# GabrieleCocco/CLFaceDetection

Measured on AMD Instinct MI355X. Metric: candidate windows/sec, 1080p, haarcascade_frontalface_alt, higher is better.
Workload: dtype u32 gathers + f32 stage sums; 1 GPU; BASELINE config 3: 64x1920x1080 8-bit frames per step in the whole job (noise/smooth/blocks mix; sharded by whole frames over 1 GPU), haarcascade_frontalface_alt, scaleFactor 1.1f, raw candidates, frames resident in HBM; frames_on_rank_0=64, windows_per_frame=6290352, parallelism=single GPU, device=AMD Radeon Graphics (gfx950:sramecc+:xnack-), 256 CUs, pipeline=vj_stream, two batches in flight

## Files before the change

### clfacedetection_amd/api.py

```python
from __future__ import annotations

import ctypes as C
import os
from dataclasses import dataclass

import numpy as np

from .build import LIB_PATH, build_lib

VJ_MAX_STAGES = 64
VJ_FLAG_COUNTERS = 1 << 0
VJ_FLAG_SIGNED_MEAN = 1 << 1
VJ_FLAG_SKIP_LIST = 1 << 2
VJ_FLAG_SKIP_ROW = 1 << 3
VJ_FLAG_GRID_F64 = 1 << 4
VJ_FLAG_TILTED_AS_UPRIGHT = 1 << 5
VJ_FLAG_CV_CANNY_PRUNING = 1 << 6
VJ_FLAG_CV_SCALE_IMAGE = 1 << 7
VJ_FLAG_CV_FIND_BIGGEST = 1 << 8
VJ_FLAG_CV_ROUGH_SEARCH = 1 << 9

CV_HAAR_DO_CANNY_PRUNING = 1
CV_HAAR_SCALE_IMAGE = 2
CV_HAAR_FIND_BIGGEST_OBJECT = 4
CV_HAAR_DO_ROUGH_SEARCH = 8

CLOD_PRECOMPUTE_FEATURES = 2 << 0
CLOD_BLOCK_IMPLEMENTATION = 2 << 1
CLOD_PER_STAGE_ITERATIONS = 2 << 2

DATA_DIR = os.path.join(os.path.dirname(os.path.abspath(__file__)), "data")


class VjError(RuntimeError):
    def __init__(self, code: int, what: str, detail: str):
        super().__init__(f"{what}: {detail}" if detail else what)
        self.code = code


class CascadeInfo(C.Structure):
    _fields_ = [(n, C.c_int32) for n in ("win_w", "win_h", "n_stages", "n_trees", "n_nodes", "n_alpha",
                                          "max_trees_per_stage", "max_nodes_per_tree", "n_tilted", "n_three_rect",
                                          "is_stump_based", "is_stage_tree")]


class Params(C.Structure):
    _fields_ = [("min_w", C.c_int32), ("min_h", C.c_int32), ("max_w", C.c_int32), ("max_h", C.c_int32),
                ("scale_factor", C.c_float), ("min_neighbors", C.c_uint32), ("flags", C.c_uint32),
                ("scale_mask", C.c_uint64 * 2)]


class ScaleInfo(C.Structure):
    _fields_ = [("scale_idx", C.c_int32), ("scale", C.c_float), ("step", C.c_float),
                ("win_w", C.c_int32), ("win_h", C.c_int32),
                ("equ_x", C.c_int32), ("equ_y", C.c_int32), ("equ_w", C.c_int32), ("equ_h", C.c_int32),
                ("area", C.c_uint32), ("nx", C.c_int32), ("ny", C.c_int32), ("accepted", C.c_int32)]


class _Image(C.Structure):
    _fields_ = [("data", C.c_void_p), ("width", C.c_int32), ("height", C.c_int32), ("stride", C.c_int32),
                ("on_device", C.c_int32), ("channels", C.c_int32)]


class CvParams(C.Structure):
    _fields_ = [("min_w", C.c_int32), ("min_h", C.c_int32), ("scale_factor", C.c_double), ("min_neighbors", C.c_uint32),
                ("flags", C.c_uint32)]


class CvPlanInfo(C.Structure):
    _fields_ = [("tile_windows", C.c_uint64), ("n_tile_scales", C.c_uint32), ("tree_prefix", C.c_uint32),
                ("tree_queue", C.c_int32), ("tq_shift", C.c_int32), ("tq_split_frames", C.c_int32), ("reserved", C.c_int32)]


class _Counters(C.Structure):
    _fields_ = [("windows", C.c_uint64), ("stump_evals", C.c_uint64), ("gather_bytes", C.c_uint64),
                ("stage_entered", C.c_uint64 * VJ_MAX_STAGES)]


VJ_MAX_PASSES = 8
VJ_MAX_LAUNCHES = 16
LAUNCH_KINDS = {0: "grid", 1: "queue", 2: "tile", 3: "block"}


class _Launch(C.Structure):
    _fields_ = [("kind", C.c_int32), ("lds_class", C.c_int32), ("stage_begin", C.c_int32), ("stage_end", C.c_int32),
                ("ms", C.c_float), ("lds_bytes", C.c_uint32), ("scale_mask", C.c_uint64 * 2),
                ("stage_entered", C.c_uint64 * VJ_MAX_STAGES)]


class _Timing(C.Structure):
    _fields_ = [("integral_ms", C.c_float), ("cascade_ms", C.c_float), ("total_ms", C.c_float),
                ("n_cascade_launches", C.c_int32), ("pass_ms", C.c_float * VJ_MAX_PASSES),
                ("pass_stage_begin", C.c_int32 * VJ_MAX_PASSES), ("pass_stage_end", C.c_int32 * VJ_MAX_PASSES),
                ("n_launches", C.c_int32), ("launch", _Launch * VJ_MAX_LAUNCHES), ("tile_split", C.c_float),
                ("balance_state", C.c_int32), ("balance_calls", C.c_int32)]


class _Result(C.Structure):
    _fields_ = [("rects", C.c_void_p), ("count", C.c_uint32), ("counters", _Counters), ("timing", _Timing)]


class CvRocParams(C.Structure):
    _fields_ = [("min_w", C.c_int32), ("min_h", C.c_int32), ("max_w", C.c_int32), ("max_h", C.c_int32),
                ("scale_factor", C.c_double), ("min_neighbors", C.c_uint32), ("flags", C.c_uint32)]


class _RocResult(C.Structure):
    _fields_ = [("r", _Result), ("reject_levels", C.c_void_p), ("level_weights", C.c_void_p)]


RECT_DTYPE = np.dtype([("x", "<i4"), ("y", "<i4"), ("w", "<i4"), ("h", "<i4"), ("weight", "<f4"),
                       ("frame", "<i4"), ("scale_idx", "<i4")])
STAGE_DTYPE = np.dtype([("first_tree", "<i4"), ("n_trees", "<i4"), ("threshold", "<f4"), ("parent", "<i4"),
                        ("next", "<i4"), ("child", "<i4")])
TREE_DTYPE = np.dtype([("first_node", "<i4"), ("n_nodes", "<i4"), ("first_alpha", "<i4")])
_RECT_DESC = np.dtype([("x", "<i4"), ("y", "<i4"), ("w", "<i4"), ("h", "<i4"), ("weight", "<f4")])
NODE_DTYPE = np.dtype([("n_rects", "<i4"), ("tilted", "<i4"), ("threshold", "<f4"), ("left", "<i4"),
                       ("right", "<i4"), ("rect", _RECT_DESC, 3)])

_SIGNATURES = {
    "vj_strerror": (C.c_char_p, [C.c_int]),
    "vj_last_error": (C.c_char_p, []),
    "vj_cascade_load_xml": (C.c_int, [C.c_char_p, C.POINTER(C.c_void_p)]),
    "vj_cascade_load": (C.c_int, [C.c_char_p, C.POINTER(C.c_void_p)]),
    "vj_cascade_save": (C.c_int, [C.c_void_p, C.c_char_p]),
    "vj_cascade_from_arrays": (C.c_int, [C.c_int, C.c_int, C.c_void_p, C.c_int, C.c_void_p, C.c_int, C.c_void_p, C.c_int,
                                         C.c_void_p, C.c_int, C.POINTER(C.c_void_p)]),
    "vj_cascade_free": (None, [C.c_void_p]),
    "vj_cascade_get_info": (C.c_int, [C.c_void_p, C.POINTER(CascadeInfo)]),
    "vj_cascade_stages": (C.c_void_p, [C.c_void_p]),
    "vj_cascade_trees": (C.c_void_p, [C.c_void_p]),
    "vj_cascade_nodes": (C.c_void_p, [C.c_void_p]),
    "vj_cascade_alpha": (C.c_void_p, [C.c_void_p]),
    "vj_cascade_notice": (C.c_char_p, [C.c_void_p]),
    "vj_params_default": (None, [C.POINTER(Params)]),
    "vj_plan_scales": (C.c_int, [C.c_void_p, C.c_int, C.c_int, C.POINTER(Params), C.POINTER(ScaleInfo), C.c_int,
                                 C.POINTER(C.c_int)]),
    "vj_plan_feature_table": (C.c_int, [C.c_void_p, C.c_int, C.POINTER(ScaleInfo), C.c_void_p, C.c_void_p]),
    "vj_env_create": (C.c_int, [C.c_int, C.POINTER(C.c_void_p)]),
    "vj_env_destroy": (None, [C.c_void_p]),
    "vj_env_reserve": (C.c_int, [C.c_void_p, C.c_int, C.c_int, C.c_int]),
    "vj_env_device_name": (C.c_int, [C.c_void_p, C.c_char_p, C.c_size_t]),
    "vj_env_configure": (C.c_int, [C.c_void_p, C.c_char_p, C.c_char_p]),
    "vj_env_query": (C.c_int, [C.c_void_p, C.c_char_p, C.c_char_p, C.c_size_t]),
    "vj_integral": (C.c_int, [C.c_void_p, C.c_void_p, C.c_int, C.c_int, C.c_int, C.c_void_p, C.c_void_p]),
    "vj_integral_image": (C.c_int, [C.c_void_p, C.c_void_p, C.c_void_p, C.c_void_p]),
    "vj_integral_tilted": (C.c_int, [C.c_void_p, C.c_void_p, C.c_void_p]),
    "vj_grayscale": (C.c_int, [C.c_void_p, C.c_void_p, C.c_void_p, C.c_int]),
    "vj_canny": (C.c_int, [C.c_void_p, C.c_void_p, C.c_void_p, C.c_int]),
    "vj_resize_linear": (C.c_int, [C.c_void_p, C.c_void_p, C.c_int, C.c_int, C.c_void_p, C.c_int]),
    "vj_host_alloc": (C.c_int, [C.c_void_p, C.c_size_t, C.POINTER(C.c_void_p)]),
    "vj_host_free": (None, [C.c_void_p, C.c_void_p]),
    "vj_detect_chain": (C.c_int, [C.c_void_p, C.c_void_p, C.c_void_p, C.POINTER(_Image), C.c_int, C.POINTER(Params),
                                  C.POINTER(Params), C.POINTER(_Result), C.POINTER(_Result)]),
    "vj_stream_create": (C.c_int, [C.c_void_p, C.c_void_p, C.c_int, C.c_int, C.c_int, C.c_int, C.POINTER(Params),
                                   C.POINTER(C.c_void_p)]),
    "vj_stream_submit": (C.c_int, [C.c_void_p, C.POINTER(_Image), C.c_int]),
    "vj_stream_collect": (C.c_int, [C.c_void_p, C.POINTER(_Result)]),
    "vj_stream_destroy": (None, [C.c_void_p]),
    "vj_detect_rois": (C.c_int, [C.c_void_p, C.c_void_p, C.POINTER(_Image), C.c_int, C.c_void_p, C.c_int, C.POINTER(Params),
                                 C.POINTER(_Result)]),
    "vj_detect_opencv": (C.c_int, [C.c_void_p, C.c_void_p, C.POINTER(_Image), C.c_int, C.POINTER(CvParams),
                                   C.POINTER(_Result)]),
    "vj_detect_opencv_rois": (C.c_int, [C.c_void_p, C.c_void_p, C.POINTER(_Image), C.c_int, C.c_void_p, C.c_int, C.POINTER(CvParams),
                                        C.POINTER(_Result)]),
    "vj_detect_opencv_chain": (C.c_int, [C.c_void_p, C.c_void_p, C.c_void_p, C.POINTER(_Image), C.c_int, C.POINTER(CvParams),
                                         C.POINTER(CvParams), C.POINTER(_Result), C.POINTER(_Result)]),
    "vj_cv_params_default": (None, [C.POINTER(CvParams)]),
    "vj_cv_roc_params_default": (None, [C.POINTER(CvRocParams)]),
    "vj_detect_opencv_roc": (C.c_int, [C.c_void_p, C.c_void_p, C.POINTER(_Image), C.c_int, C.POINTER(CvRocParams),
                                       C.POINTER(_RocResult)]),
    "vj_roc_result_free": (None, [C.POINTER(_RocResult)]),
    "vj_cv_plan_info_get": (C.c_int, [C.c_void_p, C.c_void_p, C.c_int, C.c_int, C.c_int, C.POINTER(CvParams), C.POINTER(CvPlanInfo)]),
    "vj_detect": (C.c_int, [C.c_void_p, C.c_void_p, C.POINTER(_Image), C.c_int, C.POINTER(Params),
                            C.POINTER(_Result)]),
    "vj_result_free": (None, [C.POINTER(_Result)]),
    "vj_group_rectangles": (C.c_int, [C.c_void_p, C.POINTER(C.c_uint32), C.c_int, C.c_double]),
    "vj_group_rectangles_levels": (C.c_int, [C.c_void_p, C.c_void_p, C.c_void_p, C.c_int, C.c_int, C.c_double]),
    "vj_count_windows": (C.c_int, [C.c_void_p, C.c_int, C.c_int, C.POINTER(Params), C.POINTER(C.c_uint64)]),
    "vj_shard_frames": (C.c_int, [C.c_int, C.c_int, C.c_int, C.POINTER(C.c_int), C.POINTER(C.c_int)]),
    "vj_shard_scales": (C.c_int, [C.c_void_p, C.c_int, C.c_int, C.POINTER(Params), C.c_int, C.c_int, C.POINTER(C.c_uint64)]),
}

_lib = None


def load_library(build: bool = True) -> C.CDLL:
    global _lib
    if _lib is not None:
        return _lib
    path = build_lib() if build else LIB_PATH
# ... 55 lines not shown
            return cls.load_xml(path)
        h = C.c_void_p()
        _check(load_library().vj_cascade_load(os.fsencode(path), C.byref(h)), f"vj_cascade_load({path})")
        return cls(h.value)

    @classmethod
    def from_arrays(cls, win_w: int, win_h: int, stages: np.ndarray, trees: np.ndarray, nodes: np.ndarray,
                    alpha: np.ndarray) -> "Cascade":
        st = np.ascontiguousarray(stages, STAGE_DTYPE)
        tr = np.ascontiguousarray(trees, TREE_DTYPE)
        nd = np.ascontiguousarray(nodes, NODE_DTYPE)
        al = np.ascontiguousarray(alpha, np.float32)
        h = C.c_void_p()
        _check(load_library().vj_cascade_from_arrays(int(win_w), int(win_h), st.ctypes.data, len(st), tr.ctypes.data, len(tr),
                                                     nd.ctypes.data, len(nd), al.ctypes.data, len(al), C.byref(h)),
               "vj_cascade_from_arrays")
        return cls(h.value)

    def save(self, path: str):
        _check(load_library().vj_cascade_save(self._h, os.fsencode(path)), f"vj_cascade_save({path})")

    def _view(self, fn, dtype, n):
        ptr = fn(self._h)
        buf = (C.c_char * (dtype.itemsize * n)).from_address(ptr)
        return np.frombuffer(buf, dtype, n).copy()

    @property
    def stages(self): return self._view(load_library().vj_cascade_stages, STAGE_DTYPE, self.info.n_stages)
    @property
    def trees(self): return self._view(load_library().vj_cascade_trees, TREE_DTYPE, self.info.n_trees)
    @property
    def nodes(self): return self._view(load_library().vj_cascade_nodes, NODE_DTYPE, self.info.n_nodes)
    @property
    def alpha(self): return self._view(load_library().vj_cascade_alpha, np.dtype("<f4"), self.info.n_alpha)
    @property
    def notice(self) -> str: return load_library().vj_cascade_notice(self._h).decode("latin-1")

    def plan_scales(self, width: int, height: int, params: Params | None = None) -> list[ScaleInfo]:
        p = params or default_params()
        n = C.c_int(0)
        lib = load_library()
        _check(lib.vj_plan_scales(self._h, width, height, C.byref(p), None, 0, C.byref(n)), "vj_plan_scales")
        arr = (ScaleInfo * max(n.value, 1))()
        _check(lib.vj_plan_scales(self._h, width, height, C.byref(p), arr, n.value, C.byref(n)), "vj_plan_scales")
        return list(arr)[:n.value]

    def feature_table(self, width: int, scale: ScaleInfo) -> tuple[np.ndarray, np.ndarray]:
        off = np.zeros((self.info.n_nodes, 3, 4), np.uint32)
        wts = np.zeros((self.info.n_nodes, 3), np.float32)
        _check(load_library().vj_plan_feature_table(self._h, width, C.byref(scale), off.ctypes.data,
                                                    wts.ctypes.data), "vj_plan_feature_table")
        return off, wts

    def shard_scales(self, width: int, height: int, rank: int, world: int, params: Params | None = None) -> list[int]:
        p = params or default_params()
        m = (C.c_uint64 * 2)()
        _check(load_library().vj_shard_scales(self._h, width, height, C.byref(p), world, rank, m), "vj_shard_scales")
        return [k for k in range(127) if (m[k >> 6] >> (k & 63)) & 1]

    def count_windows(self, width: int, height: int, params: Params | None = None) -> int:
        p = params or default_params()
        out = C.c_uint64(0)
        _check(load_library().vj_count_windows(self._h, width, height, C.byref(p), C.byref(out)), "vj_count_windows")
        return out.value

    def close(self):
        if self._h:
            load_library().vj_cascade_free(self._h)
            self._h = C.c_void_p()

    def __del__(self):
        try:
            self.close()
        except Exception:
            pass


@dataclass
class DetectResult:
    rects: np.ndarray
    windows: int
    stump_evals: int
    gather_bytes: int
    stage_entered: list
    integral_ms: float
    cascade_ms: float
    total_ms: float
    n_cascade_launches: int
    passes: list = None
    launches: list = None
    tile_split: float = 0.0
    balance_state: int = 0
    balance_calls: int = 0
    reject_levels: np.ndarray = None
    level_weights: np.ndarray = None

    @property
    def match_count(self) -> int:
        return len(self.rects)


class Environment:

    def __init__(self, device_index: int = 0):
        h = C.c_void_p()
        _check(load_library().vj_env_create(device_index, C.byref(h)), "vj_env_create")
# ... 379 lines not shown
```

### clfacedetection_amd/csrc/vj_env.cpp

```cpp
#include "vj_internal.hpp"
#include "vj_device.hpp"

#include <hip/hip_runtime_api.h>

#include <algorithm>
#include <climits>
#include <cmath>
#include <cstdint>
#include <cstdio>
#include <cstdlib>
#include <cstring>
#include <map>
#include <memory>
#include <string>
#include <tuple>

#include "vj_env_internal.hpp"

using namespace vj;

namespace vj {

static uint32_t f2u(float f) {
    uint32_t u;
    memcpy(&u, &f, 4);
    return u;
}

static constexpr uint32_t kSlackRows = 2;

uint32_t frame_elems_for(int W, int H) {
    uint64_t e = (uint64_t)(W + 1) * (uint64_t)(H + 1 + kSlackRows);
    e = (e + 63u) & ~(uint64_t)63u;
    return (uint32_t)e;
}

static std::vector<uint32_t> default_pass_bounds(const vj_cascade& c, const StageProgram& prog,
                                                 const std::vector<int>& override_, const std::vector<int>& cut_nodes) {
    const uint32_t n = (uint32_t)c.stages.size();
    std::vector<uint32_t> b{0};
    if (!override_.empty()) {
        for (int v : override_)
            if (v > (int)b.back() && v < (int)n) b.push_back((uint32_t)v);
    } else {
        uint32_t acc = 0;
        size_t ci = 0;
        for (uint32_t s = 0; s < n && ci < cut_nodes.size(); ++s) {
            acc += prog.n_nodes[s];
            if (acc >= (uint32_t)cut_nodes[ci] && s + 1 < n) {
                b.push_back(s + 1);
                while (ci < cut_nodes.size() && acc >= (uint32_t)cut_nodes[ci]) ++ci;
            }
        }
    }
    b.push_back(n);
    while (b.size() > (size_t)VJ_MAX_PASSES + 1) b.erase(b.end() - 2);
    return b;
}

struct TileThresholds {
    int min_windows, accept_windows, max_dwords_per_window;
};

static int build_plan(vj_env* e, const vj_cascade& c, int W, int H, const vj_params& p, Plan* pl, float tile_split,
                      const TileThresholds& thresholds, bool one_pass = false) {
    pl->tile_split = tile_split;
    if ((int)c.stages.size() > VJ_MAX_STAGES) {
        set_error("cascade has %zu stages; at most %d are supported", c.stages.size(), VJ_MAX_STAGES);
        return VJ_ERR_LIMIT;
    }
    if (!(p.flags & VJ_FLAG_TILTED_AS_UPRIGHT))
        for (const auto& nd : c.nodes)
            if (nd.tilted) {
                set_error("the cascade has tilted features: the clod profile would evaluate them as upright rectangles like the reference "
                          "(clod.cpp:448-492 never reads the flag) — pass VJ_FLAG_TILTED_AS_UPRIGHT for that, or use vj_detect_opencv");
                return VJ_ERR_UNSUPPORTED;
            }
    pl->prog = build_stage_program(c);
    const uint32_t skip_mode = p.flags & (VJ_FLAG_SKIP_LIST | VJ_FLAG_SKIP_ROW);
    pl->skip_mode = skip_mode;
    pl->pos_mode = (p.flags & VJ_FLAG_GRID_F64) ? (skip_mode == VJ_FLAG_SKIP_LIST ? 3u : 2u)
                                                : (skip_mode == VJ_FLAG_SKIP_ROW ? 1u : 0u);
    for (const auto& t : c.trees)
        if (t.n_nodes != 1) pl->trees = true;
    if (pl->trees) {
        pl->tree2 = true;
        for (const auto& t : c.trees) {
            if (t.n_nodes != 2) { pl->tree2 = false; break; }
            const vj_node_desc& n0 = c.nodes[t.first_node];
            const vj_node_desc& n1 = c.nodes[t.first_node + 1];
            const int kids = (n0.left > 0) + (n0.right > 0);
            if (kids != 1 || (n0.left > 0 ? n0.left : n0.right) != 1 || n1.left > 0 || n1.right > 0) {
                pl->tree2 = false;
                break;
            }
        }
    }
    for (size_t s = 0; s < c.stages.size(); ++s) {
        const bool linear = pl->prog.on_fail[s] == STAGE_REJECT &&
                            (pl->prog.on_pass[s] == (int)s + 1 ||
                             (pl->prog.on_pass[s] == STAGE_ACCEPT && s + 1 == c.stages.size()));
        if (!linear) pl->general = true;
    }
    std::vector<uint32_t> order;
    if (!stage_sweep_order(pl->prog, &order)) {
        set_error("stage links form a cycle");
        return VJ_ERR_UNSUPPORTED;
    }
    if (pl->general && e->general_prefix) {
        uint32_t P = 0;
        while (P + 1 < order.size() && order[P] == P && pl->prog.on_fail[P] == STAGE_REJECT &&
               pl->prog.on_pass[P] == (int)(P + 1) && order[P + 1] == P + 1)
            ++P;
        if (P >= 2) pl->general_prefix = P;
    }
    pl->scales_all = plan_scales(c, W, H, p);
    pl->frame_elems = frame_elems_for(W, H);
    const uint32_t stride = (uint32_t)W + 1u;
    const size_t n_nodes = c.nodes.size();

    uint32_t shape_header_bytes = TILE_LDS_HEADER;
    if (!pl->trees && !pl->general && e->tile_sp_begin < (int)c.stages.size()) {
        uint32_t mx = 0;
        for (size_t s = 0; s < c.stages.size(); ++s) mx = std::max(mx, pl->prog.n_nodes[s]);
        if (mx <= (uint32_t)TILE_SP_MAX_BLOCKS * TILE_SP_BLOCK) {
            pl->wave_tail = true;
            shape_header_bytes += ((2u * 14u * (TILE_SP_BLOCK + 1u) + 2u * mx + 3u) & ~3u) * 4u;
        }
    }
    const uint32_t tile_header_bytes = TILE_LDS_HEADER;
    std::vector<NodeRec> table;
    std::vector<uint32_t> pos_tab;
    std::vector<std::pair<uint32_t, uint32_t>> tile_reach;
    for (const vj_scale_info& si : pl->scales_all) {
        if (!si.accepted || si.nx <= 0 || si.ny <= 0) continue;
        if ((p.scale_mask[0] | p.scale_mask[1]) != 0) {
            const int k = si.scale_idx;
            if (k >= 127 || !((p.scale_mask[k >> 6] >> (k & 63)) & 1ull)) continue;
        }
        if (pl->scales.size() >= (size_t)MAX_SCALES) {
            set_error("more than %d scales", MAX_SCALES);
            return VJ_ERR_LIMIT;
        }
        ScaleDev sd;
        memset(&sd, 0, sizeof(sd));
        sd.step = si.step;
        sd.nx = (uint32_t)si.nx;
        sd.nwin = (uint32_t)si.nx * (uint32_t)si.ny;
        sd.e_lt = (uint32_t)si.equ_y * stride + (uint32_t)si.equ_x;
        sd.e_dw = (uint32_t)si.equ_w;
        sd.e_dh = (uint32_t)si.equ_h * stride;
        sd.area = (float)si.area;
        sd.table_first = (uint32_t)table.size();
        sd.scale_idx = (uint32_t)si.scale_idx;
        sd.scale_f = si.scale;
        sd.win_w = (uint32_t)si.win_w;
        sd.win_h = (uint32_t)si.win_h;
        sd.sq32 = e->sq32 && (uint64_t)sd.win_w * sd.win_h <= SQ32_MAX_AREA ? 1u : 0u;
        table.resize(table.size() + n_nodes);
        int rc = build_node_table(c, W, si, table.data() + sd.table_first);
        if (rc) return rc;
        const uint32_t x_max = (uint32_t)std::lrint((double)((float)(si.nx - 1) * si.step)) + (pl->pos_mode != 0u ? 1u : 0u);
        const uint32_t y_max = (uint32_t)std::lrint((double)((float)(si.ny - 1) * si.step)) + (pl->pos_mode != 0u ? 1u : 0u);
        uint32_t reach = sd.e_lt + sd.e_dh + sd.e_dw;
        for (size_t k = 0; k < n_nodes; ++k) {
            const NodeRec& r = table[sd.table_first + k];
            const uint32_t dw[3] = {r.dw01 & 0xffffu, r.dw01 >> 16, r.dw2_flags & 0xffffu};
            for (int q = 0; q < 3; ++q)
                if (q < 2 || r.w[2] != 0.0f) reach = std::max(reach, (r.lt[q] + r.dh[q] + dw[q]) / 4u);
        }
        reach += y_max * stride + x_max;
        pl->max_reach_elems = std::max(pl->max_reach_elems, reach);
        pl->windows_per_frame += sd.nwin;
        sd.ny = (uint32_t)si.ny;
        if (pl->pos_mode & 2u) {
            if (pos_tab.empty()) pos_tab.push_back(0u);
            sd.pos_base = (uint32_t)pos_tab.size();
            const double stepd = std::max(2.0, (double)si.scale);
            const int n_pos = std::max(si.nx, si.ny) + 1;
            for (int i = 0; i < n_pos; ++i)
                pos_tab.push_back((pl->pos_mode & 1u) ? (uint32_t)std::round((double)i * stepd) : (uint32_t)std::lrint((double)i * stepd));
        }

        uint32_t reach_x = (uint32_t)(si.equ_x + si.equ_w), reach_y = (uint32_t)(si.equ_y + si.equ_h);
        for (size_t k = 0; k < n_nodes; ++k) {
            const NodeRec& r = table[sd.table_first + k];
            const uint32_t dw[3] = {r.dw01 & 0xffffu, r.dw01 >> 16, r.dw2_flags & 0xffffu};
            for (int q = 0; q < 3; ++q)
                if (q < 2 || r.w[2] != 0.0f) {
                    const uint32_t lt = r.lt[q] / 4u;
                    reach_x = std::max(reach_x, lt % stride + dw[q] / 4u);
                    reach_y = std::max(reach_y, lt / stride + (r.dh[q] / 4u) / stride);
                }
        }
        if ((!pl->general || pl->general_prefix) && si.ny < 65536 && si.nx < 65536) {
            static const uint32_t kTw[] = {64, 48, 32, 24, 16, 12, 8}, kTh[] = {32, 24, 16, 12, 8, 6, 4};
            uint32_t best_cls = TILE_CLASSES, best_n = 0, b_tw = 0, b_th = 0, b_pitch = 0, b_rows = 0;
            for (uint32_t cls = 0; cls < TILE_CLASSES && best_n < (uint32_t)thresholds.min_windows; ++cls) {
                const int kb = e->tile_class_kb[cls];
                const uint32_t lds_cu = (160u - (uint32_t)e->tile_lds_reserve_kb) * 1024u;
                const uint64_t budget = kb < 0 ? ((lds_cu - 2048u) / (uint32_t)(-kb) - shape_header_bytes) & ~63ull
                                               : std::min<uint64_t>((uint64_t)kb * 1024u, 160u * 1024u - shape_header_bytes);
                for (uint32_t tw : kTw)
                    for (uint32_t th : kTh) {
                        const uint32_t nwt = tw * th;
                        if (nwt > TILE_WAVES * TILE_WAVE_CAP || nwt < 64 || nwt <= best_n) continue;
                        uint32_t pitch = (uint32_t)std::ceil((double)(tw - 1) * (double)si.step) + 3u + reach_x;
                        if (si.step != 2.0f) {
                            pitch = (pitch + 3u) & ~3u;
                            if (pitch % 32u == 0u) pitch += 4u;
                        } else {
                            pitch |= 1u;
                        }
                        const uint32_t rows = (uint32_t)std::ceil((double)(th - 1) * (double)si.step) + 3u + reach_y;
                        if ((uint64_t)pitch * rows * 4u > budget) continue;
                        if ((uint64_t)pitch * rows > (uint64_t)thresholds.max_dwords_per_window * nwt) continue;
                        best_cls = cls; best_n = nwt; b_tw = tw; b_th = th; b_pitch = pitch; b_rows = rows;
                    }
            }
            if (best_n != 0u && best_n >= (uint32_t)thresholds.accept_windows) {
                sd.tile_rw = 1;
                sd.tile_tw = b_tw;
                sd.tile_th = b_th;
                sd.tile_pitch = b_pitch;
                sd.tile_rows = b_rows;
                sd.tile_class = best_cls;
            }
        }
        if (sd.tile_rw) {
            sd.tile_table_first = (uint32_t)table.size();
            table.resize(table.size() + n_nodes);
            sd.tile_half = si.step == 2.0f ? (sd.tile_pitch + 1u) / 2u : 0u;
            if (getenv("VJ_DEBUG_PLAN"))
                fprintf(stderr, "vj plan: scale %d s=%.3f step=%.2f nx=%u ny=%u class %u tile %ux%u = %u windows, pitch %u rows %u (%u B)%s\n",
                        si.scale_idx, si.scale, si.step, sd.nx, sd.ny, sd.tile_class, sd.tile_tw, sd.tile_th, sd.tile_tw * sd.tile_th,
                        sd.tile_pitch, sd.tile_rows, sd.tile_pitch * sd.tile_rows * 4u, sd.tile_half ? " deinterleaved" : " x4");
            rc = build_node_table_stride(c, sd.tile_pitch, si, table.data() + sd.tile_table_first, sd.tile_half);
            if (rc) return rc;
            auto col = [&](uint32_t cx) { return sd.tile_half ? (cx & 1u) * sd.tile_half + (cx >> 1) : cx; };
            sd.te_lt = (uint32_t)si.equ_y * sd.tile_pitch + col((uint32_t)si.equ_x);
            sd.te_dw = (int32_t)col((uint32_t)(si.equ_x + si.equ_w)) - (int32_t)col((uint32_t)si.equ_x);
            sd.te_dh = (uint32_t)si.equ_h * sd.tile_pitch;
            sd.tiles_x = (sd.nx + sd.tile_tw - 1) / sd.tile_tw;
            sd.tile_row_end = sd.ny;
            sd.grp_table_first = sd.tile_table_first;
            sd.grp_te_lt = sd.te_lt;
            sd.grp_te_dh = sd.te_dh;
            sd.grp_te_dw = sd.te_dw;
        }
        pl->scales.push_back(sd);
        pl->scales_info.push_back(si);
        tile_reach.push_back({reach_x, reach_y});
    }
    if (pl->max_reach_elems >= pl->frame_elems) {
        set_error("feature reach %u exceeds the frame allocation %u", pl->max_reach_elems, pl->frame_elems);
        return VJ_ERR_LIMIT;
    }
    pl->tile_lead.resize(pl->scales.size());
    for (uint32_t slot = 0; slot < pl->scales.size(); ++slot) pl->tile_lead[slot] = slot;
    auto groupable = [&](uint32_t k) {
        const ScaleDev& sd = pl->scales[k];
        return sd.tile_rw != 0u && sd.tile_half != 0u && sd.step == 2.0f;
    };
    for (uint32_t g0 = 0; e->tile_group > 1 && g0 < pl->scales.size();) {
        if (!groupable(g0)) { ++g0; continue; }
        uint32_t g1 = g0 + 1;
        while (g1 < pl->scales.size() && g1 - g0 < (uint32_t)e->tile_group && groupable(g1) &&
               tile_reach[g1].first >= tile_reach[g1 - 1].first && tile_reach[g1].second >= tile_reach[g1 - 1].second)
            ++g1;
// ... 161 lines not shown
            std::vector<int> seg_first_pass;
            for (const Seg& sg : segs) {
                seg_first_pass.push_back((int)bounds.size() - 1);
                const uint32_t cut = sg.e - sg.b > 4 ? sg.b + 3 : sg.e;
                if (cut < sg.e) { bounds.push_back(cut); last.push_back(0); failq.push_back(0); }
                const uint32_t cut2 = e->seg_cut2 > 3 && sg.e - sg.b > (uint32_t)e->seg_cut2 + 4u && bounds.size() + 2 * (segs.size() - seg_first_pass.size()) + 1 < (size_t)VJ_MAX_PASSES
                                          ? sg.b + (uint32_t)e->seg_cut2 : sg.e;
                if (cut2 < sg.e) { bounds.push_back(cut2); last.push_back(0); failq.push_back(0); }
                bounds.push_back(sg.e); last.push_back(1); failq.push_back(0);
            }
            if (ok && !segs.empty() && bounds.size() - 1 <= (size_t)VJ_MAX_PASSES) {
                for (size_t k = 0; k < segs.size(); ++k) {
                    if (segs[k].fail_pos < 0) continue;
                    int target_pass = -1;
                    for (size_t t = 0; t < segs.size(); ++t)
                        if (segs[t].b == (uint32_t)segs[k].fail_pos) target_pass = seg_first_pass[t];
                    const int p_end = k + 1 < segs.size() ? seg_first_pass[k + 1] : (int)bounds.size() - 1;
                    for (int ps = seg_first_pass[k]; ps < p_end; ++ps) failq[(size_t)ps] = (uint8_t)target_pass;
                }
                pl->pass_bounds = bounds;
                pl->seg_last = last;
                pl->seg_fail = failq;
                bool chain_ok = segs.size() <= 4;
                for (size_t k = 0; k < segs.size() && chain_ok; ++k)
                    if (segs[k].fail_pos >= 0 && (k + 1 >= segs.size() || segs[k + 1].b != (uint32_t)segs[k].fail_pos)) chain_ok = false;
                if (chain_ok) {
                    pl->tile_n_seg = (uint32_t)segs.size();
                    for (size_t k = 0; k < segs.size(); ++k) {
                        pl->tile_seg_end[k] = segs[k].e;
                        if (segs[k].fail_pos >= 0) pl->tile_seg_chain |= 1u << k;
                    }
                }
            }
        }
    }
    pl->tile_end = std::min<uint32_t>((uint32_t)c.stages.size(), std::max<uint32_t>((uint32_t)e->tile_end, pl->pass_bounds[1]));
    if (pl->pass_bounds.size() == 2) pl->tile_end = pl->pass_bounds[1];
    for (uint32_t cls = 0; cls < TILE_CLASSES; ++cls) {
        pl->class_first[cls] = (uint32_t)pl->tile_units.size();
        for (uint32_t slot = 0; slot < pl->scales.size(); ++slot) {
            const uint32_t lead = pl->tile_lead[slot];
            const ScaleDev& L = pl->scales[lead];
            if (!pl->scales[slot].tile_rw || L.tile_class != cls || (slot > 0 && pl->tile_lead[slot - 1] == lead)) continue;
            uint32_t row_end = 0, nx = 0;
            for (uint32_t k = slot; k <= lead; ++k) {
                row_end = std::max(row_end, pl->scales[k].tile_row_end);
                nx = std::max(nx, pl->scales[k].nx);
            }
            for (uint32_t iy0 = 0; iy0 < row_end; iy0 += L.tile_th)
                for (uint32_t ix0 = 0; ix0 < nx; ix0 += L.tile_tw)
                    pl->tile_units.push_back(UnitDev{slot, ix0 | (iy0 << 16), lead > slot ? lead - slot + 1u : 0u, 0});
            pl->class_lds[cls] = std::max(pl->class_lds[cls], L.tile_pitch * L.tile_rows * 4u);
        }
        if (pl->class_lds[cls]) pl->class_lds[cls] += tile_header_bytes;
    }
    pl->class_first[TILE_CLASSES] = (uint32_t)pl->tile_units.size();
    const uint32_t lds_cu = (160u - (uint32_t)e->tile_lds_reserve_kb) * 1024u;
    for (uint32_t cls = 0; cls + 1 < TILE_CLASSES; ++cls) {
        const int ka = e->tile_class_kb[cls], kb = e->tile_class_kb[cls + 1];
        if (ka >= 0 || kb >= 0 || !pl->class_lds[cls] || !pl->class_lds[cls + 1]) continue;
        const uint32_t na = (uint32_t)(-ka), nb = (uint32_t)(-kb);
        if (na <= nb || na % nb != 0u) continue;
        const uint32_t ratio = na / nb;
        uint32_t big = std::max(pl->class_lds[cls + 1], ratio * pl->class_lds[cls]);
        big = (big + ratio * 1024u - 1u) / (ratio * 1024u) * (ratio * 1024u);
        if ((uint64_t)big * nb > lds_cu) continue;
        pl->class_lds[cls + 1] = big;
        pl->class_lds[cls] = big / ratio;
    }

    std::vector<UnitDev> skip_units, skip_segs;
    if (skip_mode) {
        if (pl->general) {
            set_error("the skip modes restate the reference's CPU loops, which run linear cascades only");
            return VJ_ERR_UNSUPPORTED;
        }
        uint32_t word = 0;
        for (uint32_t slot = 0; slot < pl->scales.size(); ++slot) {
            ScaleDev& sd = pl->scales[slot];
            sd.skip_base = word;
            if (skip_mode == VJ_FLAG_SKIP_ROW) {
                sd.skip_wpr = (sd.nx + 63u) / 64u;
                for (uint32_t iy = 0; iy < sd.ny; ++iy) {
                    skip_segs.push_back(UnitDev{slot, word, sd.skip_wpr, 0});
                    for (uint32_t ix0 = 0; ix0 < sd.nx; ix0 += 64u)
                        skip_units.push_back(UnitDev{slot, ix0 | (iy << 16), std::min<uint32_t>(64u, sd.nx - ix0), word++});
                }
            } else {
                sd.skip_wpr = 0;
                const uint32_t n_words = (sd.nwin + 63u) / 64u;
                skip_segs.push_back(UnitDev{slot, word, n_words, 0});
                for (uint32_t i0 = 0; i0 < sd.nwin; i0 += 64u)
                    skip_units.push_back(UnitDev{slot, i0, std::min<uint32_t>(64u, sd.nwin - i0), word++});
            }
        }
        pl->skip_frame_words = word;
        pl->n_skip_units = (uint32_t)skip_units.size();
        pl->n_skip_segs = (uint32_t)skip_segs.size();
    }

    int rc;
    if (!skip_units.empty()) {
        if ((rc = pl->d_skip_units.ensure(skip_units.size() * sizeof(UnitDev)))) return rc;
        if ((rc = pl->d_skip_segs.ensure(skip_segs.size() * sizeof(UnitDev)))) return rc;
        HIP_TRY(hipMemcpy(pl->d_skip_units.p, skip_units.data(), skip_units.size() * sizeof(UnitDev), hipMemcpyHostToDevice));
        HIP_TRY(hipMemcpy(pl->d_skip_segs.p, skip_segs.data(), skip_segs.size() * sizeof(UnitDev), hipMemcpyHostToDevice));
    }
    if ((rc = pl->d_table.ensure(std::max<size_t>(table.size(), 1) * sizeof(NodeRec)))) return rc;
    if ((rc = pl->d_scales.ensure(std::max<size_t>(pl->scales.size(), 1) * sizeof(ScaleDev)))) return rc;
    if ((rc = pl->d_stages.ensure(pl->stages.size() * sizeof(StageDev)))) return rc;
    if ((rc = pl->d_units.ensure(std::max<size_t>(pl->units.size(), 1) * sizeof(UnitDev)))) return rc;
    if ((rc = pl->d_tile_units.ensure(std::max<size_t>(pl->tile_units.size(), 1) * sizeof(UnitDev)))) return rc;
    if (!pos_tab.empty()) {
        if ((rc = pl->d_pos_tab.ensure(pos_tab.size() * sizeof(uint32_t)))) return rc;
        HIP_TRY(hipMemcpy(pl->d_pos_tab.p, pos_tab.data(), pos_tab.size() * sizeof(uint32_t), hipMemcpyHostToDevice));
    }
    if (!pl->unit_groups.empty()) {
        if ((rc = pl->d_unit_groups.ensure(pl->unit_groups.size() * sizeof(UnitDev)))) return rc;
        HIP_TRY(hipMemcpy(pl->d_unit_groups.p, pl->unit_groups.data(), pl->unit_groups.size() * sizeof(UnitDev), hipMemcpyHostToDevice));
    }
    if ((rc = pl->d_sp_blocks.ensure(std::max<size_t>(sp_blocks.size(), 1) * sizeof(SpBlock)))) return rc;
    if (!sp_blocks.empty())
        HIP_TRY(hipMemcpy(pl->d_sp_blocks.p, sp_blocks.data(), sp_blocks.size() * sizeof(SpBlock), hipMemcpyHostToDevice));
    if (!pl->tile_units.empty())
        HIP_TRY(hipMemcpy(pl->d_tile_units.p, pl->tile_units.data(), pl->tile_units.size() * sizeof(UnitDev),
                          hipMemcpyHostToDevice));
    if (!table.empty())
        HIP_TRY(hipMemcpy(pl->d_table.p, table.data(), table.size() * sizeof(NodeRec), hipMemcpyHostToDevice));
    HIP_TRY(hipMemcpy(pl->d_stages.p, pl->stages.data(), pl->stages.size() * sizeof(StageDev), hipMemcpyHostToDevice));
    if (!pl->units.empty())
        HIP_TRY(hipMemcpy(pl->d_units.p, pl->units.data(), pl->units.size() * sizeof(UnitDev), hipMemcpyHostToDevice));
    return VJ_OK;
}

static int layout_queues(Plan* pl, int frames, uint64_t* total_entries) {
    const uint64_t frames_per_part = frames >= (int)Q_PARTS ? ((uint64_t)frames + Q_PARTS - 1) / Q_PARTS : 1;
    uint64_t base = 0;
    for (ScaleDev& sd : pl->scales) {
        sd.q_base = (uint32_t)base;
        sd.q_cap = (uint32_t)((uint64_t)sd.nwin * frames_per_part);
        base += (uint64_t)sd.nwin * frames_per_part * std::min<uint64_t>(Q_PARTS, (uint64_t)frames);
    }
    *total_entries = base;
    if (base > 0xffffffffull) {
        set_error("survivor queue needs %llu entries", (unsigned long long)base);
        return VJ_ERR_LIMIT;
    }
    if (pl->frames_q != frames && !pl->scales.empty()) {
        HIP_TRY(hipMemcpy(pl->d_scales.p, pl->scales.data(), pl->scales.size() * sizeof(ScaleDev),
                          hipMemcpyHostToDevice));
        pl->frames_q = frames;
    }
    return VJ_OK;
// ... 137 lines not shown
    FILE* f = fopen(path, "w");
    if (!f) {
        set_error("cannot write %s", path);
        return VJ_ERR_IO;
    }
    for (const auto& kv : e->balance) {
        const vj_env::PlanKey& k = std::get<0>(kv.first);
        const vj_env::Balance& b = kv.second;
        fprintf(f, "vjbal1 %llx %d %d %d %d %d %d %x %llx %llx %x %d %.4f %d %d %u %u %d\n", (unsigned long long)std::get<0>(k), std::get<1>(k),
                std::get<2>(k), std::get<3>(k), std::get<4>(k), std::get<5>(k), std::get<6>(k), std::get<7>(k), (unsigned long long)std::get<8>(k),
                (unsigned long long)std::get<9>(k), std::get<10>(k), std::get<1>(kv.first), (double)b.best, b.phase == 4 ? 0 : b.thr, b.phase,
                b.calls_total, b.calls_on_candidate, b.calls);
    }
    fclose(f);
    return VJ_OK;
}

static int balance_import(vj_env* e, const char* path) {
    FILE* f = fopen(path, "r");
    if (!f) {
        set_error("cannot read %s", path);
        return VJ_ERR_IO;
    }
    char line[512];
    int n_bad = 0;
    while (fgets(line, sizeof(line), f)) {
        unsigned long long hash, m0, m1;
        int W, H, a, b2, c2, d, cls, thr, state = 3;
        unsigned sf, flags;
        double split;
        if (line[0] == '#' || line[0] == '\n') continue;
        if (sscanf(line, "vjbal1 %llx %d %d %d %d %d %d %x %llx %llx %x %d %lf %d %d", &hash, &W, &H, &a, &b2, &c2, &d, &sf, &m0, &m1, &flags, &cls,
                   &split, &thr, &state) < 14 || !(split >= 0.0 && split <= 3.0) || cls < 1) {
            ++n_bad;
            continue;
        }
        if (state == 0) continue;
        vj_env::Balance b;
        b.cur = b.best = (float)split;
        b.thr = thr ? 1 : 0;
        b.phase = 3;
        b.thr_tried = b.far_tried = true;
        b.last_used = ++e->balance_tick;
        e->balance[vj_env::BalanceKey(vj_env::PlanKey((uint64_t)hash, W, H, a, b2, c2, d, (uint32_t)sf, (uint64_t)m0, (uint64_t)m1, (uint32_t)flags, 0u), cls)] = b;
    }
    fclose(f);
    if (n_bad) {
        set_error("%s: %d lines are not balance records", path, n_bad);
        return VJ_ERR_PARSE;
    }
    return VJ_OK;
}

static int get_plan(vj_env* e, const vj_cascade* c, int W, int H, const vj_params& p, Plan** out, int n_frames = 1 << 20) {
    const vj_env::Balance* bal = balance_of(e, c, W, H, p, n_frames, false);
    const BalanceChoice choice = bal ? balance_choice(bal, n_frames) : BalanceChoice{e->split_for(n_frames, p), 0, false};
    const float split = choice.split;
    int small = small_frame_class(e, W, H, n_frames);
    if (small == 0 && choice.thr == 1 && !e->tile_thresholds_set) small = 3;
    const bool one_pass = n_frames <= e->one_pass_max_frames && (uint64_t)W * (uint64_t)H >= 800000ull;
    vj_env::PlanKey key(c->uid, W, H, p.min_w, p.min_h, p.max_w, p.max_h, f2u(p.scale_factor), p.scale_mask[0],
                        p.scale_mask[1], (p.flags & (VJ_FLAG_SKIP_LIST | VJ_FLAG_SKIP_ROW | VJ_FLAG_GRID_F64 | VJ_FLAG_TILTED_AS_UPRIGHT)) | ((uint32_t)small << 8) | ((uint32_t)one_pass << 12), f2u(split));
    auto it = e->plans.find(key);
    if (it != e->plans.end()) {
        it->second->last_used = ++e->plan_tick;
        *out = it->second.get();
        return VJ_OK;
    }
    if ((int)e->plans.size() >= std::max(2, e->plan_cache_max)) {
        HIP_TRY(hipStreamSynchronize(e->stream));
        if (e->stream2) HIP_TRY(hipStreamSynchronize(e->stream2));
        while ((int)e->plans.size() >= std::max(2, e->plan_cache_max)) {
            auto lru = e->plans.begin();
            for (auto i = e->plans.begin(); i != e->plans.end(); ++i)
                if (i->second->last_used < lru->second->last_used) lru = i;
            lru->second->release_device();
            e->plans.erase(lru);
        }
    }
    auto pl = std::make_unique<Plan>();
    TileThresholds th{e->tile_min_windows, e->tile_accept_windows, e->tile_max_dwords_per_window};
    if (small == 2) th = TileThresholds{64, 64, 8000};
    else if (small == 1) th = TileThresholds{256, 256, 2000};
    else if (small == 3) th = TileThresholds{std::min(384, th.min_windows), std::min(384, th.accept_windows), th.max_dwords_per_window};
    int rc = build_plan(e, *c, W, H, p, pl.get(), split, th, one_pass);
    if (rc) {
        pl->release_device();
        return rc;
    }
    pl->last_used = ++e->plan_tick;
    *out = pl.get();
    e->plans[key] = std::move(pl);
    return VJ_OK;
}

int Lane::create() {
    for (auto& x : ev) HIP_TRY(hipEventCreate(&x));
    for (auto& x : pass_ev) HIP_TRY(hipEventCreate(&x));
    for (auto& x : launch_ev) HIP_TRY(hipEventCreate(&x));
    HIP_TRY(hipEventCreateWithFlags(&upload_done, hipEventDisableTiming));
    HIP_TRY(hipEventCreateWithFlags(&integral_done, hipEventDisableTiming));
    HIP_TRY(hipEventCreateWithFlags(&done, hipEventDisableTiming));
    h_pinned_bytes = (size_t)1 << 20;
    HIP_TRY(hipHostMalloc(&h_pinned, h_pinned_bytes, hipHostMallocDefault));
    return VJ_OK;
}

void Lane::destroy() {
    for (DevBuf* b : {&d_gray, &d_counts, &d_det}) b->release();
    if (h_pinned) (void)hipHostFree(h_pinned);
    if (h_stage) (void)hipHostFree(h_stage);
    h_pinned = h_stage = nullptr;
    for (auto& x : ev) if (x) (void)hipEventDestroy(x);
    for (auto& x : pass_ev) if (x) (void)hipEventDestroy(x);
    for (auto& x : launch_ev) if (x) (void)hipEventDestroy(x);
    for (hipEvent_t* x : {&upload_done, &integral_done, &done}) if (*x) (void)hipEventDestroy(*x);
}

int ensure_image_buffers(vj_env* e, int W, int H, int frames, bool need_gray, int channels, Lane* lane) {
    if (!lane) lane = &e->lane0;
    const size_t fe = frame_elems_for(W, H);
    const uint32_t n_bands = ((uint32_t)H + BAND_ROWS - 1) / BAND_ROWS;
    const uint32_t band_pitch = ((uint32_t)W + 3u) & ~3u;
    int rc;
    const size_t sum_bytes = fe * 4 * (size_t)frames, sq_bytes = fe * 8 * (size_t)frames;
    const bool grow = sum_bytes > e->d_sum.cap || sq_bytes > e->d_sqsum.cap;
    if ((rc = e->d_sum.ensure(sum_bytes))) return rc;
    if ((rc = e->d_sqsum.ensure(sq_bytes))) return rc;
    (void)grow;
    if (need_gray) {
        const size_t gstride = ((size_t)W * (size_t)channels + 3) & ~(size_t)3;
        if ((rc = lane->d_gray.ensure(gstride * (size_t)H * (size_t)frames))) return rc;
    }
    const size_t band_elems = (size_t)frames * n_bands * band_pitch;
    if ((rc = e->d_band_sum.ensure(band_elems * 4))) return rc;
    if ((rc = e->d_band_sq.ensure(band_elems * 4))) return rc;
    if ((rc = e->d_band_sqp.ensure(band_elems * 8))) return rc;
    return VJ_OK;
// ... 1870 lines not shown
    vj_env* e = s->e;
    HIP_TRY(hipSetDevice(e->device));
    const int lane = s->n_pending == 0 ? 0 : 1 - s->fifo[0];
    Lane* L = &s->lanes[lane];
    HIP_TRY(hipEventSynchronize(L->integral_done));
    if ((rc = enqueue_prepare(e, L, s->plan.get(), frames, n_frames, W, H, true, s->copy))) return rc;
    if ((rc = enqueue_cascade(e, L, s->plan.get(), W, H, s->p))) return rc;
    s->fifo[s->n_pending] = lane;
    s->n_frames_of[lane] = n_frames;
    s->n_pending++;
    return VJ_OK;
}

int vj_stream_collect(vj_stream* s, vj_result* out) {
    if (!s || !out) return VJ_ERR_ARG;
    memset(out, 0, sizeof(*out));
    if (s->n_pending == 0) {
        set_error("no batch is pending");
        return VJ_ERR_ARG;
    }
    vj_env* e = s->e;
    HIP_TRY(hipSetDevice(e->device));
    const int lane = s->fifo[0];
    s->fifo[0] = s->fifo[1];
    s->n_pending--;
    Lane* L = &s->lanes[lane];
    std::vector<RawDet> dets;
    int rc = finish_batch(e, L, s->plan.get(), 0, s->W, s->H, s->p, &dets, &out->counters, &out->timing);
    if (rc) return rc;
    return build_result(s->plan.get(), dets, s->n_frames_of[lane], s->p, out);
}

void vj_stream_destroy(vj_stream* s) {
    if (!s) return;
    (void)hipSetDevice(s->e->device);
    if (s->e->stream) (void)hipStreamSynchronize(s->e->stream);
    if (s->e->stream2) (void)hipStreamSynchronize(s->e->stream2);
    if (s->copy) {
        (void)hipStreamSynchronize(s->copy);
        (void)hipStreamDestroy(s->copy);
    }
    for (Lane& L : s->lanes) L.destroy();
    if (s->plan) s->plan->release_device();
    delete s;
}

void vj_result_free(vj_result* r) {
    if (!r) return;
    free(r->rects);
    r->rects = nullptr;
    r->count = 0;
}

}
```

### include/vj.h

```cpp
#ifndef VJ_H_
#define VJ_H_

#include <stdint.h>
#include <stddef.h>

#ifdef __cplusplus
extern "C" {
#endif
#if defined(VJ_BUILDING) && defined(__GNUC__)
#pragma GCC visibility push(default)
#endif

enum {
    VJ_OK = 0,
    VJ_ERR_ARG = 1,
    VJ_ERR_IO = 2,
    VJ_ERR_PARSE = 3,
    VJ_ERR_UNSUPPORTED = 4,
    VJ_ERR_NO_DEVICE = 5,
    VJ_ERR_HIP = 6,
    VJ_ERR_NOMEM = 7,
    VJ_ERR_LIMIT = 8
};
const char* vj_strerror(int code);
// ... 32 lines not shown
int  vj_cascade_load_xml(const char* path, vj_cascade** out);
int  vj_cascade_load(const char* path, vj_cascade** out);
int  vj_cascade_save(const vj_cascade* c, const char* path);
int  vj_cascade_from_arrays(int win_w, int win_h, const vj_stage_desc* stages, int n_stages,
                            const vj_tree_desc* trees, int n_trees, const vj_node_desc* nodes, int n_nodes,
                            const float* alpha, int n_alpha, vj_cascade** out);
void vj_cascade_free(vj_cascade* c);
int  vj_cascade_get_info(const vj_cascade* c, vj_cascade_info* out);
const vj_stage_desc* vj_cascade_stages(const vj_cascade* c);
const vj_tree_desc*  vj_cascade_trees(const vj_cascade* c);
const vj_node_desc*  vj_cascade_nodes(const vj_cascade* c);
const float*         vj_cascade_alpha(const vj_cascade* c);
const char*          vj_cascade_notice(const vj_cascade* c);

enum {
    VJ_FLAG_COUNTERS     = 1u << 0,
    VJ_FLAG_SIGNED_MEAN  = 1u << 1,
    VJ_FLAG_SKIP_LIST    = 1u << 2,
    VJ_FLAG_SKIP_ROW     = 1u << 3,
    VJ_FLAG_GRID_F64     = 1u << 4,
    VJ_FLAG_TILTED_AS_UPRIGHT = 1u << 5,
    VJ_FLAG_CV_CANNY_PRUNING = 1u << 6,
    VJ_FLAG_CV_SCALE_IMAGE = 1u << 7,
    VJ_FLAG_CV_FIND_BIGGEST = 1u << 8,
    VJ_FLAG_CV_ROUGH_SEARCH = 1u << 9,
};

typedef struct vj_params {
    int32_t  min_w, min_h;
    int32_t  max_w, max_h;
    float    scale_factor;
    uint32_t min_neighbors;
    uint32_t flags;
    uint64_t scale_mask[2];
} vj_params;
#define VJ_SCALE_MASK_NONE (1ull << 63)
void vj_params_default(vj_params* p);

typedef struct vj_scale_info {
    int32_t  scale_idx;
    float    scale;
    float    step;
    int32_t  win_w, win_h;
    int32_t  equ_x, equ_y, equ_w, equ_h;
    uint32_t area;
    int32_t  nx, ny;
    int32_t  accepted;
} vj_scale_info;
int vj_plan_scales(const vj_cascade* c, int width, int height, const vj_params* p,
                   vj_scale_info* out, int cap, int* n);

int vj_plan_feature_table(const vj_cascade* c, int width, const vj_scale_info* s,
                          uint32_t* offsets, float* weights);

typedef struct vj_env vj_env;
int  vj_env_create(int device_index, vj_env** out);
void vj_env_destroy(vj_env* e);
int  vj_env_reserve(vj_env* e, int max_w, int max_h, int max_batch);
int  vj_env_device_name(const vj_env* e, char* buf, size_t cap);
int  vj_env_configure(vj_env* e, const char* key, const char* value);
int  vj_env_query(const vj_env* e, const char* key, char* buf, size_t cap);

int vj_integral(vj_env* e, const uint8_t* gray, int w, int h, int stride,
                uint32_t* sum, uint64_t* sqsum);

int  vj_host_alloc(vj_env* e, size_t bytes, void** out);
void vj_host_free(vj_env* e, void* p);

struct vj_image;
int  vj_integral_image(vj_env* e, const struct vj_image* image, uint32_t* sum, uint64_t* sqsum);
int  vj_grayscale(vj_env* e, const struct vj_image* image, uint8_t* gray, int gray_stride);
int  vj_integral_tilted(vj_env* e, const struct vj_image* image, uint32_t* tilted);
int  vj_canny(vj_env* e, const struct vj_image* image, uint8_t* edges, int edges_stride);
int  vj_resize_linear(vj_env* e, const struct vj_image* image, int dst_w, int dst_h, uint8_t* dst, int dst_stride);
typedef struct vj_image {
    const uint8_t* data;
    int32_t width, height;
    int32_t stride;
    int32_t on_device;
    int32_t channels;
} vj_image;

typedef struct vj_rect {
    int32_t x, y, w, h;
    float   weight;
    int32_t frame;
    int32_t scale_idx;
} vj_rect;

#define VJ_MAX_STAGES 64
typedef struct vj_counters {
    uint64_t windows;
    uint64_t stump_evals;
    uint64_t gather_bytes;
    uint64_t stage_entered[VJ_MAX_STAGES];
} vj_counters;

#define VJ_MAX_PASSES 8
#define VJ_MAX_LAUNCHES 16
enum { VJ_LAUNCH_GRID = 0,
       VJ_LAUNCH_QUEUE = 1,
       VJ_LAUNCH_TILE = 2,
       VJ_LAUNCH_BLOCK = 3 };
typedef struct vj_launch {
    int32_t  kind;
    int32_t  lds_class;
// ... 106 lines not shown
```

Before: 10.47 billion windows/s.

## Widen LDS tile shape search and drop wave-tail header from tile budget

```diff
diff --git a/clfacedetection_amd/api.py b/clfacedetection_amd/api.py
--- a/clfacedetection_amd/api.py
+++ b/clfacedetection_amd/api.py
@@ -55,6 +55,22 @@
                 ("win_w", C.c_int32), ("win_h", C.c_int32),
                 ("equ_x", C.c_int32), ("equ_y", C.c_int32), ("equ_w", C.c_int32), ("equ_h", C.c_int32),
                 ("area", C.c_uint32), ("nx", C.c_int32), ("ny", C.c_int32), ("accepted", C.c_int32)]
+
+
+class TileInfo(C.Structure):
+    _fields_ = [("scale_idx", C.c_int32), ("scale", C.c_float), ("step", C.c_float), ("nx", C.c_int32), ("ny", C.c_int32),
+                ("lds_class", C.c_int32), ("tile_w", C.c_int32), ("tile_h", C.c_int32), ("pitch", C.c_int32), ("rows", C.c_int32),
+                ("reach_x", C.c_int32), ("reach_y", C.c_int32), ("lead_scale_idx", C.c_int32), ("tile_row_end", C.c_int32)]
+
+
+class TilePlanInfo(C.Structure):
+    _fields_ = [("header_bytes", C.c_uint32), ("gather_reserve_bytes", C.c_uint32), ("max_tile_windows", C.c_uint32),
+                ("n_classes", C.c_uint32), ("class_lds", C.c_uint32 * 4), ("class_per_cu", C.c_int32 * 4),
+                ("class_tiles", C.c_uint32 * 4)]
+
+
+VJ_PLAN_TILES_FORMER_SHAPES = 1
+VJ_PLAN_TILES_NO_GROUPS = 2
 
 
 class _Image(C.Structure):
@@ -137,6 +153,8 @@
     "vj_plan_scales": (C.c_int, [C.c_void_p, C.c_int, C.c_int, C.POINTER(Params), C.POINTER(ScaleInfo), C.c_int,
                                  C.POINTER(C.c_int)]),
     "vj_plan_feature_table": (C.c_int, [C.c_void_p, C.c_int, C.POINTER(ScaleInfo), C.c_void_p, C.c_void_p]),
+    "vj_plan_tiles": (C.c_int, [C.c_void_p, C.c_int, C.c_int, C.POINTER(Params), C.c_int, C.c_uint32, C.POINTER(TilePlanInfo),
+                                C.POINTER(TileInfo), C.c_int, C.POINTER(C.c_int)]),
     "vj_env_create": (C.c_int, [C.c_int, C.POINTER(C.c_void_p)]),
     "vj_env_destroy": (None, [C.c_void_p]),
     "vj_env_reserve": (C.c_int, [C.c_void_p, C.c_int, C.c_int, C.c_int]),
@@ -298,6 +316,18 @@
                                                     wts.ctypes.data), "vj_plan_feature_table")
         return off, wts
 
+    def plan_tiles(self, width: int, height: int, n_frames: int = 64, params: Params | None = None,
+                   flags: int = 0) -> tuple[TilePlanInfo, list[TileInfo]]:
+        p = params or default_params()
+        n = C.c_int(0)
+        info = TilePlanInfo()
+        lib = load_library()
+        _check(lib.vj_plan_tiles(self._h, width, height, C.byref(p), n_frames, flags, None, None, 0, C.byref(n)), "vj_plan_tiles")
+        arr = (TileInfo * max(n.value, 1))()
+        _check(lib.vj_plan_tiles(self._h, width, height, C.byref(p), n_frames, flags, C.byref(info), arr, n.value, C.byref(n)),
+               "vj_plan_tiles")
+        return info, list(arr)[:n.value]
+
     def shard_scales(self, width: int, height: int, rank: int, world: int, params: Params | None = None) -> list[int]:
         p = params or default_params()
         m = (C.c_uint64 * 2)()
diff --git a/clfacedetection_amd/csrc/vj_env.cpp b/clfacedetection_amd/csrc/vj_env.cpp
--- a/clfacedetection_amd/csrc/vj_env.cpp
+++ b/clfacedetection_amd/csrc/vj_env.cpp
@@ -62,8 +62,14 @@
     int min_windows, accept_windows, max_dwords_per_window;
 };
 
-static int build_plan(vj_env* e, const vj_cascade& c, int W, int H, const vj_params& p, Plan* pl, float tile_split,
-                      const TileThresholds& thresholds, bool one_pass = false) {
+struct PlanBuildOptions {
+    bool upload = true;
+    bool former_shapes = false;
+    std::vector<std::pair<uint32_t, uint32_t>>* tile_reach = nullptr;
+};
+
+static int build_plan(const vj_env* e, const vj_cascade& c, int W, int H, const vj_params& p, Plan* pl, float tile_split,
+                      const TileThresholds& thresholds, bool one_pass = false, const PlanBuildOptions& opt = PlanBuildOptions()) {
     pl->tile_split = tile_split;
     if ((int)c.stages.size() > VJ_MAX_STAGES) {
         set_error("cascade has %zu stages; at most %d are supported", c.stages.size(), VJ_MAX_STAGES);
@@ -119,16 +125,16 @@
     const uint32_t stride = (uint32_t)W + 1u;
     const size_t n_nodes = c.nodes.size();
 
-    uint32_t shape_header_bytes = TILE_LDS_HEADER;
+    const uint32_t tile_header_bytes = TILE_LDS_HEADER;
+    uint32_t shape_header_bytes = tile_header_bytes;
     if (!pl->trees && !pl->general && e->tile_sp_begin < (int)c.stages.size()) {
         uint32_t mx = 0;
         for (size_t s = 0; s < c.stages.size(); ++s) mx = std::max(mx, pl->prog.n_nodes[s]);
         if (mx <= (uint32_t)TILE_SP_MAX_BLOCKS * TILE_SP_BLOCK) {
             pl->wave_tail = true;
-            shape_header_bytes += ((2u * 14u * (TILE_SP_BLOCK + 1u) + 2u * mx + 3u) & ~3u) * 4u;
-        }
-    }
-    const uint32_t tile_header_bytes = TILE_LDS_HEADER;
+            if (opt.former_shapes) shape_header_bytes += ((2u * 14u * (TILE_SP_BLOCK + 1u) + 2u * mx + 3u) & ~3u) * 4u;
+        }
+    }
     std::vector<NodeRec> table;
     std::vector<uint32_t> pos_tab;
     std::vector<std::pair<uint32_t, uint32_t>> tile_reach;
@@ -194,7 +200,8 @@
                 }
         }
         if ((!pl->general || pl->general_prefix) && si.ny < 65536 && si.nx < 65536) {
-            static const uint32_t kTw[] = {64, 48, 32, 24, 16, 12, 8}, kTh[] = {32, 24, 16, 12, 8, 6, 4};
+            static const uint32_t kTw[] = {64, 56, 48, 40, 32, 24, 16, 12, 8}, kTh[] = {32, 28, 24, 20, 16, 12, 8, 6, 4};
+            auto former = [&](uint32_t v) { return opt.former_shapes && (v == 56u || v == 40u || v == 28u || v == 20u); };
             uint32_t best_cls = TILE_CLASSES, best_n = 0, b_tw = 0, b_th = 0, b_pitch = 0, b_rows = 0;
             for (uint32_t cls = 0; cls < TILE_CLASSES && best_n < (uint32_t)thresholds.min_windows; ++cls) {
                 const int kb = e->tile_class_kb[cls];
@@ -204,7 +211,8 @@
                 for (uint32_t tw : kTw)
                     for (uint32_t th : kTh) {
                         const uint32_t nwt = tw * th;
-                        if (nwt > TILE_WAVES * TILE_WAVE_CAP || nwt < 64 || nwt <= best_n) continue;
+                        if (nwt > TILE_WAVES * TILE_WAVE_CAP || nwt < 64 || nwt < best_n || (nwt == best_n && best_cls != cls)) continue;
+                        if (former(tw) || former(th)) continue;
                         uint32_t pitch = (uint32_t)std::ceil((double)(tw - 1) * (double)si.step) + 3u + reach_x;
                         if (si.step != 2.0f) {
                             pitch = (pitch + 3u) & ~3u;
@@ -215,6 +223,7 @@
                         const uint32_t rows = (uint32_t)std::ceil((double)(th - 1) * (double)si.step) + 3u + reach_y;
                         if ((uint64_t)pitch * rows * 4u > budget) continue;
                         if ((uint64_t)pitch * rows > (uint64_t)thresholds.max_dwords_per_window * nwt) continue;
+                        if (nwt == best_n && (opt.former_shapes || pitch * rows >= b_pitch * b_rows)) continue;
                         best_cls = cls; best_n = nwt; b_tw = tw; b_th = th; b_pitch = pitch; b_rows = rows;
                     }
             }
@@ -482,6 +491,9 @@
                     pl->tile_units.push_back(UnitDev{slot, ix0 | (iy0 << 16), lead > slot ? lead - slot + 1u : 0u, 0});
             pl->class_lds[cls] = std::max(pl->class_lds[cls], L.tile_pitch * L.tile_rows * 4u);
         }
+        for (const ScaleDev& sd : pl->scales)
+            if (sd.tile_rw && sd.tile_class == cls && pl->class_lds[cls])
+                pl->class_lds[cls] = std::max(pl->class_lds[cls], sd.tile_pitch * sd.tile_rows * 4u);
         if (pl->class_lds[cls]) pl->class_lds[cls] += tile_header_bytes;
     }
     pl->class_first[TILE_CLASSES] = (uint32_t)pl->tile_units.size();
@@ -529,6 +541,8 @@
         pl->n_skip_segs = (uint32_t)skip_segs.size();
     }
 
+    if (opt.tile_reach) *opt.tile_reach = tile_reach;
+    if (!opt.upload) return VJ_OK;
     int rc;
     if (!skip_units.empty()) {
         if ((rc = pl->d_skip_units.ensure(skip_units.size() * sizeof(UnitDev)))) return rc;
@@ -772,6 +786,14 @@
     return VJ_OK;
 }
 
+static TileThresholds thresholds_for(const vj_env* e, int small) {
+    TileThresholds th{e->tile_min_windows, e->tile_accept_windows, e->tile_max_dwords_per_window};
+    if (small == 2) th = TileThresholds{64, 64, 8000};
+    else if (small == 1) th = TileThresholds{256, 256, 2000};
+    else if (small == 3) th = TileThresholds{std::min(384, th.min_windows), std::min(384, th.accept_windows), th.max_dwords_per_window};
+    return th;
+}
+
 static int get_plan(vj_env* e, const vj_cascade* c, int W, int H, const vj_params& p, Plan** out, int n_frames = 1 << 20) {
     const vj_env::Balance* bal = balance_of(e, c, W, H, p, n_frames, false);
     const BalanceChoice choice = bal ? balance_choice(bal, n_frames) : BalanceChoice{e->split_for(n_frames, p), 0, false};
@@ -799,11 +821,7 @@
         }
     }
     auto pl = std::make_unique<Plan>();
-    TileThresholds th{e->tile_min_windows, e->tile_accept_windows, e->tile_max_dwords_per_window};
-    if (small == 2) th = TileThresholds{64, 64, 8000};
-    else if (small == 1) th = TileThresholds{256, 256, 2000};
-    else if (small == 3) th = TileThresholds{std::min(384, th.min_windows), std::min(384, th.accept_windows), th.max_dwords_per_window};
-    int rc = build_plan(e, *c, W, H, p, pl.get(), split, th, one_pass);
+    int rc = build_plan(e, *c, W, H, p, pl.get(), split, thresholds_for(e, small), one_pass);
     if (rc) {
         pl->release_device();
         return rc;
@@ -2780,4 +2798,61 @@
     r->count = 0;
 }
 
-}
+int vj_plan_tiles(const vj_cascade* c, int width, int height, const vj_params* p, int n_frames, uint32_t flags,
+                  vj_tile_plan_info* info, vj_tile_info* out, int cap, int* n) {
+    if (!c || !p || !n || width <= 0 || height <= 0 || n_frames <= 0 || (cap > 0 && !out) ||
+        (flags & ~(uint32_t)(VJ_PLAN_TILES_FORMER_SHAPES | VJ_PLAN_TILES_NO_GROUPS)))
+        return VJ_ERR_ARG;
+    int rc = check_params(*p);
+    if (rc) return rc;
+    auto e = std::make_unique<vj_env>();
+    if (flags & VJ_PLAN_TILES_NO_GROUPS) e->tile_group = 1;
+    Plan pl;
+    PlanBuildOptions opt;
+    std::vector<std::pair<uint32_t, uint32_t>> reach;
+    opt.upload = false;
+    opt.former_shapes = (flags & VJ_PLAN_TILES_FORMER_SHAPES) != 0u;
+    opt.tile_reach = &reach;
+    const bool one_pass = n_frames <= e->one_pass_max_frames && (uint64_t)width * (uint64_t)height >= 800000ull;
+    rc = build_plan(e.get(), *c, width, height, *p, &pl, e->split_for(n_frames, *p),
+                    thresholds_for(e.get(), small_frame_class(e.get(), width, height, n_frames)), one_pass, opt);
+    if (rc) return rc;
+    if (info) {
+        memset(info, 0, sizeof(*info));
+        info->header_bytes = TILE_LDS_HEADER;
+        info->gather_reserve_bytes = (uint32_t)e->tile_lds_reserve_kb * 1024u;
+        info->max_tile_windows = TILE_WAVES * TILE_WAVE_CAP;
+        info->n_classes = TILE_CLASSES;
+        for (uint32_t cls = 0; cls < TILE_CLASSES; ++cls) {
+            info->class_lds[cls] = pl.class_lds[cls];
+            info->class_per_cu[cls] = e->tile_class_kb[cls] < 0 ? -e->tile_class_kb[cls] : 0;
+            info->class_tiles[cls] = pl.class_first[cls + 1] - pl.class_first[cls];
+        }
+    }
+    *n = (int)pl.scales.size();
+    for (int k = 0; k < *n && k < cap; ++k) {
+        const ScaleDev& sd = pl.scales[(size_t)k];
+        vj_tile_info& t = out[k];
+        memset(&t, 0, sizeof(t));
+        t.scale_idx = (int32_t)sd.scale_idx;
+        t.scale = sd.scale_f;
+        t.step = sd.step;
+        t.nx = (int32_t)sd.nx;
+        t.ny = (int32_t)sd.ny;
+        t.reach_x = (int32_t)reach[(size_t)k].first;
+        t.reach_y = (int32_t)reach[(size_t)k].second;
+        t.lds_class = -1;
+        t.lead_scale_idx = t.scale_idx;
+        if (!sd.tile_rw) continue;
+        t.lds_class = (int32_t)sd.tile_class;
+        t.tile_w = (int32_t)sd.tile_tw;
+        t.tile_h = (int32_t)sd.tile_th;
+        t.pitch = (int32_t)sd.tile_pitch;
+        t.rows = (int32_t)sd.tile_rows;
+        t.lead_scale_idx = (int32_t)pl.scales[pl.tile_lead[(size_t)k]].scale_idx;
+        t.tile_row_end = (int32_t)sd.tile_row_end;
+    }
+    return VJ_OK;
+}
+
+}
diff --git a/include/vj.h b/include/vj.h
--- a/include/vj.h
+++ b/include/vj.h
@@ -108,6 +108,31 @@
 
 int vj_plan_feature_table(const vj_cascade* c, int width, const vj_scale_info* s,
                           uint32_t* offsets, float* weights);
+
+typedef struct vj_tile_info {
+    int32_t  scale_idx;
+    float    scale, step;
+    int32_t  nx, ny;
+    int32_t  lds_class;
+    int32_t  tile_w, tile_h;
+    int32_t  pitch, rows;
+    int32_t  reach_x, reach_y;
+    int32_t  lead_scale_idx;
+    int32_t  tile_row_end;
+} vj_tile_info;
+typedef struct vj_tile_plan_info {
+    uint32_t header_bytes;
+    uint32_t gather_reserve_bytes;
+    uint32_t max_tile_windows;
+    uint32_t n_classes;
+    uint32_t class_lds[4];
+    int32_t  class_per_cu[4];
+    uint32_t class_tiles[4];
+} vj_tile_plan_info;
+#define VJ_PLAN_TILES_FORMER_SHAPES 1u
+#define VJ_PLAN_TILES_NO_GROUPS     2u
+int vj_plan_tiles(const vj_cascade* c, int width, int height, const vj_params* p, int n_frames,
+                  uint32_t flags, vj_tile_plan_info* info, vj_tile_info* out, int cap, int* n);
 
 typedef struct vj_env vj_env;
 int  vj_env_create(int device_index, vj_env** out);
```

New measurement: 10.63 billion windows/s (median of 6 runs). 1.5% higher.
